# NWC-CUAHSI-Summer-Institute/LGAR-py

Measured on AMD Instinct MI355X. Metric: column-timesteps/sec, higher is better.
Workload: dtype f32

## Files before the change

### lgar_py_amd/csrc/lgar_column.hpp

```cpp
#pragma once
#include "lgar_geff.hpp"

namespace lgar {

template <typename R> struct Glob {
  R dt_h, initial_psi, pdm, wp_psi, frozen;
  R giuh[LGAR_GMAX];
  int nint, nsub, ng, bottom_mode, closed_form;
  long long iter_cap;
};

#define LGAR_COOP_GROUPS 16
template <typename S, int FMAX, int STRIDE = WAVE> struct FrontsView {
  S *base;
  unsigned char *fl;
  __device__ __forceinline__ S &Z(int i) const { return base[(0 * FMAX + i) * STRIDE]; }
  __device__ __forceinline__ S &TH(int i) const { return base[(1 * FMAX + i) * STRIDE]; }
  __device__ __forceinline__ S &PS(int i) const { return base[(2 * FMAX + i) * STRIDE]; }
  __device__ __forceinline__ S &DZ(int i) const { return base[(3 * FMAX + i) * STRIDE]; }
  __device__ __forceinline__ unsigned char &flag(int i) const { return fl[i * STRIDE]; }
  __device__ __forceinline__ int layer(int i) const { return fl[i * STRIDE] & 0x7f; }
  __device__ __forceinline__ bool bottom(int i) const { return (fl[i * STRIDE] & LGAR_FLAG_BOTTOM) != 0; }
  __device__ __forceinline__ void set_flag(int i, int layer, bool bottom) const {
    fl[i * STRIDE] = (unsigned char)(layer | (bottom ? LGAR_FLAG_BOTTOM : 0));
  }
  __device__ __forceinline__ void copy(int dst, int src) const {
    Z(dst) = Z(src); TH(dst) = TH(src); PS(dst) = PS(src); DZ(dst) = DZ(src);
    fl[dst * STRIDE] = fl[src * STRIDE];
  }
};

constexpr int MODE_LITERAL = 0, MODE_FAST = 1, MODE_MIXED = 3, MODE_COOP = 4, MODE_MIXED_COOP = 6;

template <typename S, int MODE> struct ModeTraits : ScalarKind<S> {
  using K = ScalarKind<S>;
  static constexpr bool literal = MODE == MODE_LITERAL;
  static constexpr bool mixed = MODE == MODE_MIXED || MODE == MODE_MIXED_COOP;
  static constexpr bool coop = MODE == MODE_COOP || MODE == MODE_MIXED_COOP;
  static constexpr bool mixed_f64 = mixed && K::plain_f64;
  static constexpr bool coop_f64 = coop && K::plain_f64;
  static constexpr int pol = (literal && K::f64) ? POL_LIBRARY : (!literal && K::plain_f32) ? POL_RCP32 : mixed_f64 ? POL_MIXED : POL_LEAN;
  static constexpr int stride = coop ? LGAR_COOP_GROUPS : WAVE;
  static constexpr bool giuh_mem = MODE == MODE_MIXED && !K::dual;
  static constexpr bool late_forcing_sums = MODE == MODE_MIXED;
  static constexpr bool fused_walk = !literal && !coop;
};

template <typename S, int NL, int FMAX, int MODE> struct Column {
  using R = real_t<S>;
  using M = ModeTraits<S, MODE>;
  static constexpr int POL = M::pol;
  const ColParams<S, NL> &P;
  const LGAR_KARG Glob<R> *G;
  FrontsView<S, FMAX, M::stride> F;
  int nf;
  int status;
  S ponded_water, previous_precip, ending_volume;
  S giuh_q[LGAR_GMAX];
  static constexpr int DEAD = LGAR_ST_BOTTOM | LGAR_ST_OVERFLOW | LGAR_ST_STRUCT;
  R *giuh_mem = nullptr;
  size_t giuh_stride = 0;
  bool giuh_live = false;
  S k_deepest;
  bool new_front_frozen;
  S memo_theta, memo_g;
  int memo_layer = -1;
  unsigned near_sat_fronts = 0u;
  S post_mass;
  bool post_mass_valid = false;
  bool post_event = false;
  bool psi_rewritten = false;
  S aet_psi_wp_memo;
  bool aet_psi_wp_known = false;
  bool count_geff = false;
  int share_lanes = 0;
  R *xchg = nullptr;
  int coop_rank = 0;
  int cap = FMAX;
  S a_precip, a_pet, a_aet, a_infil, a_runoff, a_perc, a_giuh, a_disch;

  __device__ Column(const ColParams<S, NL> &p, const LGAR_KARG Glob<R> *g, const FrontsView<S, FMAX, M::stride> &f) : P(p), G(g), F(f) {}

  __device__ __forceinline__ S cum_at(int k) const { return sel<S, NL>(P.cum, k); }
  __device__ __forceinline__ S capillary_drive(const LayerK<S> &lk, S theta1, S theta2, int site = 0, CoopRiders *riders = nullptr) {
    (void)site; (void)riders;
    LGAR_MEASURE_POINT(NOGEFF, lk, theta1, theta2)
    LGAR_COUNT_GEFF_CALL(site)
    LGAR_MEASURE_POINT(DUP_GEFF, lk, theta1, theta2)
    if constexpr (M::literal && M::f64) {
      return G->closed_form ? geff_closed<S, POL>(lk, theta1, theta2) : geff_literal<S, POL>(lk, theta1, theta2, G->nint);
    }
    if constexpr (M::dual && M::f64 && !M::literal) {
      if (share_lanes >= 2 && !G->closed_form) return geff_fused<S>(lk, theta1, theta2, G->nint, xchg, share_lanes);
    }
    if constexpr (M::coop_f64 && !M::mixed) {
      if (share_lanes > 1 && !G->closed_form) return geff_fused<S>(lk, theta1, theta2, G->nint, xchg, share_lanes, coop_rank, riders);
    }
    if constexpr (M::coop_f64 && M::mixed) {
      if (share_lanes > 1 && !G->closed_form)
        return geff_mixed_coop(val(lk.alpha), val(lk.n), val(lk.m), val(lk.inv_m), val(lk.inv_n), val(lk.ksat), val(lk.te), val(lk.tr),
                               theta1, theta2, G->nint, xchg, share_lanes, coop_rank);
    }
    if constexpr (M::mixed_f64) {
      if (!G->closed_form)
        return geff_mixed(val(lk.alpha), val(lk.n), val(lk.m), val(lk.inv_m), val(lk.inv_n), val(lk.ksat), val(lk.te), val(lk.tr),
                          theta1, theta2, G->nint);
    }
#ifndef LGAR_NO_F32_RARE_GEFF
    if constexpr (M::plain_f32 && !M::literal) {
      if (site != 1 && !G->closed_form)
        return geff_f32_rare(lk.alpha, lk.n, lk.m, lk.inv_m, lk.inv_n, lk.te, lk.tr, theta1, theta2, G->nint);
    }
#endif
    return G->closed_form ? geff_closed<S, POL>(lk, theta1, theta2) : geff(lk, theta1, theta2, G->nint);
  }
  __device__ __forceinline__ double capillary_drive_fronts(const LayerK<double> &lk, double theta1, double theta2, double psi1,
                                                           double psi2, double &kr_end) {
    LGAR_MEASURE_POINT(NOGEFF_FRONTS, lk, theta1, theta2, kr_end)
    LGAR_COUNT_GEFF_CALL(1)
    if constexpr (M::coop && M::mixed) {
      if (share_lanes > 1) return geff_mixed_heads<true>(lk, theta1, theta2, psi1, psi2, G->nint, kr_end, xchg, share_lanes, coop_rank);
    }
    return geff_mixed_heads(lk, theta1, theta2, psi1, psi2, G->nint, kr_end);
  }
  __device__ __forceinline__ S cum_prev(int k) const {
    S r = S(R(0.0));
#pragma unroll
    for (int j = 0; j < NL - 1; j++) {
      const S cj = P.cum[j];
      r = choose(k == j + 1, cj, r);
    }
    return r;
  }

  __device__ __forceinline__ bool feq(int a, int b) const {
    return val(F.Z(a)) == val(F.Z(b)) && val(F.PS(a)) == val(F.PS(b)) && val(F.DZ(a)) == val(F.DZ(b));
  }
  __device__ __forceinline__ void fdel(int i) {
    for (int j = i; j < nf - 1; j++) F.copy(j, j + 1);
    nf--;
  }
  __device__ __forceinline__ void range_of(int k, int &lo, int &len) const {
    lo = -1; len = 0;
    for (int i = 0; i < nf; i++)
      if (F.layer(i) == k) { if (len == 0) lo = i; len++; }
  }

  static constexpr int SCAN = 8;
  struct Rows {
    R z[SCAN], th[SCAN];
    int fl[SCAN];
  };
  __device__ __forceinline__ void fetch_rows(Rows &r) const {
#pragma unroll
    for (int q = 0; q < SCAN; q++) {
      r.z[q] = val(F.Z(q));
      r.th[q] = val(F.TH(q));
      r.fl[q] = F.flag(q);
    }
  }

  __device__ __forceinline__ S mass_balance() const {
    S ls[NL];
    if constexpr (M::coop_f64) {
      if (nf <= SCAN) {
        Rows r;
        fetch_rows(r);
#pragma unroll
        for (int j = 0; j < NL; j++) ls[j] = S(R(0.0));
#pragma unroll
        for (int q = 0; q < SCAN; q++) {
          const bool on = q < nf;
          const int lay = r.fl[q] & 0x7f;
          const bool next_same = (q + 1 < nf) && ((r.fl[(q + 1 < SCAN) ? q + 1 : q] & 0x7f) == lay);
          const R dth = next_same ? r.th[q] - r.th[(q + 1 < SCAN) ? q + 1 : q] : r.th[q];
          R base = R(0.0);
#pragma unroll
          for (int j = 1; j < NL; j++) base = choose(lay == j, val(P.cum[j]) - val(P.thick[j]), base);
          const R term = (r.z[q] - base) * dth;
#pragma unroll
          for (int j = 0; j < NL; j++) ls[j] = choose(on && lay == j, ls[j] + term, ls[j]);
        }
        S tot = ls[NL - 1];
#pragma unroll
        for (int j = NL - 2; j >= 0; j--) tot = ls[j] + tot;
        return tot;
      }
    }
    int i = 0;
#pragma unroll
    for (int j = 0; j < NL; j++) {
      S base = (j == 0) ? S(R(0.0)) : P.cum[j] - P.thick[j];
      S sum = S(R(0.0));
      while (i < nf && F.layer(i) == j) {
        bool next_same = (i + 1 < nf) && (F.layer(i + 1) == j);
        S dth = next_same ? (F.TH(i) - F.TH(i + 1)) : F.TH(i);
        sum = sum + (F.Z(i) - base) * dth;
        i++;
      }
      ls[j] = sum;
    }
    S tot = ls[NL - 1];
#pragma unroll
    for (int j = NL - 2; j >= 0; j--) tot = ls[j] + tot;
    return tot;
  }

  __device__ __forceinline__ S mass_and_events(bool &ev) const {
    S ls[NL];
    bool e = false;
    int i = 0;
#pragma unroll
    for (int j = 0; j < NL; j++) {
      S base = (j == 0) ? S(R(0.0)) : P.cum[j] - P.thick[j];
      S sum = S(R(0.0));
      while (i < nf && F.layer(i) == j) {
        const bool has_next = i + 1 < nf;
        const int fn = has_next ? F.flag(i + 1) : 0;
        const bool next_same = has_next && ((fn & 0x7f) == j);
        const S zi = F.Z(i), ti = F.TH(i);
        if (has_next) {
          const S zn = F.Z(i + 1), tn = F.TH(i + 1);
          e = e || (next_same && !(fn & LGAR_FLAG_BOTTOM) && val(zi) > val(zn));
          e = e || (next_same && val(ti) <= val(tn));
          e = e || (val(zi) > val(P.cum[j]));
          sum = sum + (zi - base) * (next_same ? (ti - tn) : ti);
        } else {
          sum = sum + (zi - base) * ti;
        }
        i++;
      }
      ls[j] = sum;
    }
    S tot = ls[NL - 1];
#pragma unroll
    for (int j = NL - 2; j >= 0; j--) tot = ls[j] + tot;
    ev = e;
    return tot;
  }

  __device__ __forceinline__ int free_drainage_front() const {
    R psi = val(F.PS(0));
    int idx = 0;
    for (int i = 0; i < nf; i++) {
      R pi = val(F.PS(i));
      if (pi <= psi) { psi = pi; idx = i; }
      else if (ab(pi - psi) <= R(1e-8) + R(1e-5) * ab(psi)) { psi = pi; idx = i; }
    }
    return idx;
  }

  __device__ __forceinline__ static void theta_slope(R alpha, R n, R m, R te, R tr, R psi, R &th, R &dth) {
    R ap = pwp<POL>(alpha * psi, n);
    R one_ap = R(1.0) + ap;
    R op = pwp<POL>(one_ap, m);
    R span = dv<POL>(R(1.0), op) * (te - tr);
    th = span + tr;
    dth = (psi > R(0.0)) ? dv<POL>(-(span * m * n * ap), psi * one_ap) : R(0.0);
  }

  __device__ __forceinline__ static void theta_slope2(R alpha, R n, R m, R te, R tr, R psi, R &th, R &dth, R &d2th) {
    R ap = pwp<POL>(alpha * psi, n);
    R one_ap = R(1.0) + ap;
    R op = pwp<POL>(one_ap, m);
    R span = dv<POL>(R(1.0), op) * (te - tr);
    th = span + tr;
    const R r = (psi > R(0.0)) ? dv<POL>(R(1.0), psi * one_ap) : R(0.0);
    dth = -(span * m * n * ap) * r;
    d2th = dth * ((n - R(1.0)) - n * ap) * r;
  }

  struct FirstEval {
    bool have = false;
    R M = R(0.0), dM = R(0.0), d2M = R(0.0);
    R thk = R(0.0);
    __device__ __forceinline__ void add(R thick, R th, R below, R dth, R d2th) {
      M += thick * (th - below);
      dM += thick * dth;
      d2M += thick * d2th;
    }
  };

  template <int K>
  __device__ __forceinline__ S theta_mass_balance_newton_f32(const LayerK<S> &lk, S psi0, S new_mass, S prior_mass,
                                                             const S (&dth)[NL], const S (&dthick)[NL], S dth_k, S dthick_k) {
// ... 464 lines not shown
          S psi_old = oc_ps;
          S psi = F.PS(i);
          S base = P.cum[NL - 2];
          S prior_mass = (oc_z - base) * (oc_th - R(0.0));
          S new_mass = (z - base) * (F.TH(i) - R(0.0));
          FirstEval fe;
#pragma unroll
          for (int j = 0; j < NL - 1; j++) {
            const LayerK<S> lj = pick_static(P, j);
            if constexpr (M::f64) {
              S theta;
              if constexpr (!M::dual) {
                R th, dt, d2;
                theta_slope2(val(lj.alpha), val(lj.n), val(lj.m), val(lj.te), val(lj.tr), val(psi), th, dt, d2);
                fe.add(val(P.thick[j]), th, R(0.0), dt, d2);
                theta = S(th);
              } else {
                theta = theta_from_h<S, POL>(lj, psi);
              }
              prior_mass = prior_mass + P.thick[j] * (theta - R(0.0));
              new_mass = new_mass + P.thick[j] * (theta - R(0.0));
            } else {
              S theta_old = theta_from_h<S, POL>(lj, psi_old);
              prior_mass = prior_mass + P.thick[j] * (theta_old - R(0.0));
              S theta = theta_from_h<S, POL>(lj, psi);
              new_mass = new_mass + P.thick[j] * (theta - R(0.0));
            }
            dthick[j] = P.thick[j];
          }
          if constexpr (M::plain_f64) {
            R tk, dk, ek;
            theta_slope2(val(lk.alpha), val(lk.n), val(lk.m), val(lk.te), val(lk.tr), val(psi), tk, dk, ek);
            fe.add(val(z) - val(base), tk, R(0.0), dk, ek);
            fe.thk = tk;
            fe.have = true;
          }
          if (F.layer(c.fdd) == NL - 1) prior_mass = prior_mass + c.infiltration - (R(0.0) + c.aet);
          S theta_new = theta_mass_balance<NL - 1>(lk, psi, new_mass, prior_mass, dth, dthick, S(R(0.0)), z - base, fe);
          F.TH(i) = mn(theta_new, lk.te);
          need_psi = true;
        }
      }
      if (need_psi) F.PS(i) = h_from_se<S, POL>(lk, se_from_theta(lk, F.TH(i)));
      LGAR_MEASURE_POINT(CLK, 24)
      c.on_z = oc_z; c.on_th = oc_th; c.on_ps = oc_ps;
      c.i = i - 1;
    }
  }
  template <int K> __device__ __forceinline__ void sweep_from(SweepCarry &c) {
    sweep_layer<K>(c);
    if constexpr (K > 0) sweep_from<K - 1>(c);
  }

  __device__ __forceinline__ void move_sweep(S infiltration, S aet, S old_mass, int fdd) {
    SweepCarry c;
    c.i = nf - 1; c.nf0 = nf; c.fdd = fdd;
    c.infiltration = infiltration; c.aet = aet;
    c.on_z = c.on_th = c.on_ps = S(R(0.0));
    c.near_sat = 0u;
    sweep_from<NL - 1>(c);
    near_sat_fronts = c.near_sat;
    if constexpr (!M::fused_walk) {
      check_column_mass(fdd, old_mass, infiltration, aet);
    } else {
      const S theta_e_k1 = sel<S, NL>(P.te, F.layer(fdd));
      const S mass_timestep = (old_mass + infiltration) - (aet + R(0.0));
      bool stepped = false, literal = false;
      if (__builtin_expect(ab(val(F.TH(fdd)) - val(theta_e_k1)) < Tol<R>::mass, 0)) {
        const S current_mass = mass_balance();
        const R err = ab(val(current_mass) - val(mass_timestep));
        if (ab(err - Tol<R>::mass) > Tol<R>::mass) {
          const bool nxt_same = (fdd + 1 < nf) && (F.layer(fdd + 1) == F.layer(fdd));
          const R slope = nxt_same ? val(F.TH(fdd)) - val(F.TH(fdd + 1)) : val(F.TH(fdd));
          if (slope > R(0.0)) {
            F.Z(fdd) = F.Z(fdd) + dv<POL>(val(mass_timestep) - val(current_mass), slope);
            stepped = true;
          } else {
            literal = true;
          }
        }
      }
      if (__builtin_expect(literal, 0)) check_column_mass(fdd, old_mass, infiltration, aet);
      post_mass = mass_and_events(post_event);
      if (stepped) {
        const R err = ab(val(post_mass) - val(mass_timestep));
        if (__builtin_expect(ab(err - Tol<R>::mass) > Tol<R>::mass, 0)) {
          check_column_mass(fdd, old_mass, infiltration, aet);
          post_mass = mass_and_events(post_event);
        }
      }
      post_mass_valid = true;
    }
  }

  __device__ __forceinline__ void merge_fronts() {
    int i = 0, lo = 0;
    while (i < nf - 1) {
      const int k = F.layer(i);
      if (i > 0 && F.layer(i - 1) != k) lo = i;
      const int nx = i + 1;
      const bool passing = (val(F.Z(i)) > val(F.Z(nx))) && (F.layer(nx) == k) && !F.bottom(nx);
      if (!passing) { i++; continue; }
      const int nn = i + 2;
      if (nn >= nf) { status |= LGAR_ST_STRUCT; return; }
      const LayerK<S> lk = pick(P, k);
      S mass = F.Z(i) * (F.TH(i) - F.TH(nx)) + F.Z(nx) * (F.TH(nx) - F.TH(nn));
      F.Z(i) = mass / (F.TH(i) - F.TH(nn));
      S se = se_from_theta(lk, F.TH(i));
      F.PS(i) = h_from_se<S, POL>(lk, se);
      int j = lo;
      while (j < nf && F.layer(j) == k && !feq(j, nx)) j++;
      if (j < nf && F.layer(j) == k) fdel(j);
      i = lo;
      while (i < nf && F.layer(i) == k) i++;
      lo = i;
    }
  }

  __device__ __forceinline__ void cross_layer_boundary() {
    int i = 0;
    while (i < nf - 1) {
      const int k = F.layer(i);
      const int nx = i + 1, nn = i + 2;
      const S cumk = cum_at(k);
      if (!(val(F.Z(i)) > val(cumk) && val(F.Z(nx)) == val(cumk))) { i++; continue; }
      if (k == NL - 1) {
        if (G->bottom_mode == 0) { status |= LGAR_ST_BOTTOM; return; }
        i++;
        continue;
      }
      if (nn >= nf) { status |= LGAR_ST_STRUCT; return; }
      const LayerK<S> lk = pick(P, k);
      const LayerK<S> ln = pick(P, k + 1);
      S overshot = F.Z(i) - F.Z(nx);
      S se = se_from_theta(lk, F.TH(i));
      F.PS(i) = h_from_se<S, POL>(lk, se);
// ... 73 lines not shown
#pragma unroll
    for (int j = NL - 2; j >= 0; j--) tot = ls[j] + tot;
    return tot;
  }

  __device__ __forceinline__ void update_psi() {
    for (int i = 0; i < nf - 1; i++) {
      const LayerK<S> lk = pick(P, F.layer(i));
      F.PS(i) = h_from_se<S, POL>(lk, se_from_theta(lk, F.TH(i)));
    }
  }

  __device__ __forceinline__ S front_k(int i, const LayerK<S> &lk) const {
    S k = k_from_se<S, POL>(lk, se_from_theta(lk, F.TH(i)));
    if (i == 0 && new_front_frozen) k = k * G->frozen;
    return k;
  }

  __device__ __forceinline__ bool front_event_pending() const {
    bool ev = false;
    S z1 = F.Z(0), t1 = F.TH(0);
    int f1 = F.flag(0);
    for (int i = 0; i + 1 < nf; i++) {
      const S z2 = F.Z(i + 1), t2 = F.TH(i + 1);
      const int f2 = F.flag(i + 1);
      const bool same = ((f1 ^ f2) & 0x7f) == 0;
      ev = ev || (same && !(f2 & LGAR_FLAG_BOTTOM) && val(z1) > val(z2));
      ev = ev || (same && val(t1) <= val(t2));
      ev = ev || (val(z1) > val(cum_at(f1 & 0x7f)));
      z1 = z2; t1 = t2; f1 = f2;
    }
    return ev;
  }

  __device__ __forceinline__ S move_wetting_front(S infiltration, S &aet, S old_mass, int fdd) {
    move_sweep(infiltration, aet, old_mass, fdd);
    LGAR_MEASURE_POINT(CLK, 3)
    S bottom_flux = S(R(0.0));
    LGAR_MEASURE_POINT(DUP_EVENT)
    bool pending;
    if constexpr (M::fused_walk) pending = post_event;
    else pending = front_event_pending();
    if (__builtin_expect(pending, 0)) {
      post_mass_valid = false;
      psi_rewritten = false;
      for (int pass = 0; pass < 2; pass++) {
        merge_fronts();
        if (pass == 0) cross_layer_boundary();
      }
      if (G->bottom_mode != 0) bottom_flux = cross_domain_boundary();
      S mass_change = fix_dry_over_wet();
      if (ab(val(mass_change)) > R(1e-7)) aet = aet - mass_change;
      if constexpr (!M::literal) { if (psi_rewritten || near_sat_fronts != 0u) update_psi(); }
    } else if constexpr (!M::literal && M::f64) {
      if (__builtin_expect(near_sat_fronts != 0u, 0)) {
        for (int i = 0; i < nf - 1; i++)
          if (near_sat_fronts & (1u << i)) {
            const LayerK<S> lk = pick(P, F.layer(i));
            F.PS(i) = h_from_se<S, POL>(lk, se_from_theta(lk, F.TH(i)));
          }
      }
    }
    if constexpr (M::literal) update_psi();
    LGAR_MEASURE_POINT(CLK, 4)
    LGAR_MEASURE_POINT(DUP_PSI)
    return bottom_flux;
  }

  __device__ __forceinline__ int calc_dzdt_pairs(S h_p) {
    const int hl = share_lanes >> 1;
    const bool upper = coop_rank >= hl;
    const int r2 = upper ? coop_rank - hl : coop_rank;
    R *tab2 = xchg + (upper ? LGAR_COOP_TAB_ROW : 0);
    int i = -1;
    auto next_moving = [&]() {
      while (++i < nf - 1) {
        if (F.bottom(i)) { F.DZ(i) = S(R(0.0)); continue; }
        const bool top = F.layer(i) == 0;
        if (top && val(F.TH(i + 1)) > val(F.TH(i))) status |= LGAR_ST_THETA_ORDER;
        if (val(F.TH(i) - F.TH(i + 1)) > R(0.0)) return i;
        F.DZ(i) = S(R(0.0));
      }
      return -1;
    };
    for (;;) {
      const int ia = next_moving();
      if (ia < 0) return i;
      const int ib = next_moving();
      const int ka = F.layer(ia), kb = (ib >= 0) ? F.layer(ib) : 0;
      if (ib < 0 || hl < 5 + ((ka > kb) ? ka : kb)) return ia - 1;
      const int im = upper ? ib : ia;
      const int k = upper ? kb : ka;
      const LayerK<S> lk = pick(P, k);
      const S theta_1 = F.TH(im + 1), theta_2 = F.TH(im);
      CoopRiders riders;
      {
        const int e = r2 - 5;
        LayerK<S> le = lk;
        S th_e = theta_2;
#pragma unroll
        for (int j = 0; j < NL - 1; j++) {
          const bool mine = (e == j) && (j < k);
          le.alpha = choose(mine, P.alpha[j], le.alpha); le.n = choose(mine, P.n[j], le.n); le.m = choose(mine, P.m[j], le.m);
          le.inv_m = choose(mine, P.inv_m[j], le.inv_m); le.ksat = choose(mine, P.ksat[j], le.ksat);
          le.te = choose(mine, P.te[j], le.te); le.tr = choose(mine, P.tr[j], le.tr);
        }
// ... 79 lines not shown
      const LayerK<S> lk = pick(P, k);
      LGAR_COUNT_GEFF_CALL(1)
      LGAR_COUNT_GEFF_CALL(1)
      double kr_mine;
      const S g_mine = geff_mixed_heads<true>(lk, F.TH(im + 1), F.TH(im), F.PS(im + 1), F.PS(im), G->nint, kr_mine, tab2, hl, r2);
      tab2[0] = g_mine;
      tab2[1] = kr_mine;
#pragma unroll
      for (int j = 0; j < NL - 1; j++)
        if (j < kmax) {
          const LayerK<S> lj = pick_static(P, j);
          const S tl = theta_from_h<S, POL>(lj, F.PS(im));
          tab2[2 + j] = k_from_se<S, POL>(lj, se_from_theta(lj, tl));
        }
      lds_exchange_point();
      S g2[2];
      R kr2[2], kk[2][NL];
#pragma unroll
      for (int h = 0; h < 2; h++) {
        g2[h] = xchg[h * 64];
        kr2[h] = xchg[h * 64 + 1];
#pragma unroll
        for (int j = 0; j < NL - 1; j++) kk[h][j] = xchg[h * 64 + 2 + j];
      }
      lds_exchange_point();
#pragma unroll
      for (int h = 0; h < 2; h++) {
        const int f = h ? ib : ia;
        const int kf = h ? kb : ka;
        const LayerK<S> lf = pick(P, kf);
        const S g = g2[h];
        S ki = lf.ksat * kr2[h];
        if (f == 0 && new_front_frozen) ki = ki * G->frozen;
        if (is_nan(val(g))) status |= LGAR_ST_NAN;
        const S delta_theta = F.TH(f) - F.TH(f + 1);
        S dzdt;
        if (kf == 0) {
          dzdt = dv<POL>(S(R(1.0)), delta_theta) * (dv<POL>(lf.ksat * (g + h_p), F.Z(f)) + ki);
        } else {
          S den = S(R(0.0)) + dv<POL>(F.Z(f) - cum_prev(kf), ki);
#pragma unroll
          for (int j = 0; j < NL - 1; j++)
            if (j < kf) {
              S pt = (j != 0) ? P.cum[(j > 0) ? j - 1 : 0] : S(R(0.0));
              den = den + dv<POL>(P.cum[j] - pt, S(kk[h][j]));
            }
          dzdt = dv<POL>(S(R(1.0)), delta_theta) * (dv<POL>(F.Z(f), den) + dv<POL>(lf.ksat * (g + h_p), F.Z(f)));
        }
        F.DZ(f) = dzdt;
      }
    }
  }

  __device__ __forceinline__ void calc_dzdt(S h_p) {
    int i = -1;
    if constexpr (M::coop_f64 && M::mixed) {
      if (share_lanes >= 4 && !G->closed_form) i = calc_dzdt_pairs_mixed(h_p);
    }
    if constexpr (M::coop_f64 && !M::mixed) {
      if (share_lanes >= LGAR_COOP_PAIR_LANES && !G->closed_form) i = calc_dzdt_pairs(h_p);
    }
    for (;;) {
      bool found = false;
      while (!found && ++i < nf - 1) {
        if (F.bottom(i)) { F.DZ(i) = S(R(0.0)); continue; }
        const bool top = F.layer(i) == 0;
        if (top && val(F.TH(i + 1)) > val(F.TH(i))) status |= LGAR_ST_THETA_ORDER;
        if (val(F.TH(i) - F.TH(i + 1)) > R(0.0)) found = true;
        else F.DZ(i) = S(R(0.0));
      }
      if (any_lane(found) == 0ull) break;
      LGAR_MEASURE_POINT(CLK, 10)
      if (found) {
        const int k = F.layer(i);
        const LayerK<S> lk = pick(P, k);
        S theta_1 = F.TH(i + 1), theta_2 = F.TH(i);
        S delta_theta = F.TH(i) - F.TH(i + 1);
        S g, ki;
        bool fronts_done = false;
        if constexpr (M::mixed_f64) {
          if (!G->closed_form) {
            double kr_end;
            g = capillary_drive_fronts(lk, theta_1, theta_2, F.PS(i + 1), F.PS(i), kr_end);
            ki = lk.ksat * kr_end;
            if (i == 0 && new_front_frozen) ki = ki * G->frozen;
            fronts_done = true;
          }
        }
        CoopRiders riders;
        if constexpr (M::coop_f64 && !M::mixed) {
          if (!G->closed_form && share_lanes >= 5 + k) {
            const int e = coop_rank - 5;
            LayerK<S> le = lk;
            S th_e = F.TH(i);
            if (k > 0) {
#pragma unroll
              for (int j = 0; j < NL - 1; j++) {
                const bool mine = (e == j) && (j < k);
                le.alpha = choose(mine, P.alpha[j], le.alpha); le.n = choose(mine, P.n[j], le.n); le.m = choose(mine, P.m[j], le.m);
                le.inv_m = choose(mine, P.inv_m[j], le.inv_m); le.ksat = choose(mine, P.ksat[j], le.ksat);
                le.te = choose(mine, P.te[j], le.te); le.tr = choose(mine, P.tr[j], le.tr);
              }
              const S tl = theta_from_h<S, POL>(le, F.PS(i));
              th_e = choose(e >= 0 && e < k, tl, th_e);
            }
            riders.n = 1 + k;
            riders.l = le;
// ... 171 lines not shown
  }

  __device__ __forceinline__ void drain() {
    a_precip = a_pet = a_aet = a_infil = a_runoff = a_perc = a_giuh = a_disch = S(R(0.0));
  }

  __device__ __forceinline__ void forward(S precip, S pet) {
    const R dt = G->dt_h;
    if (is_nan(val(precip)) || is_nan(val(pet))) status |= LGAR_ST_NAN;
    S ending_volume_sub = ending_volume;
    for (int sub = 0; sub < G->nsub; sub++) {
      if (status & DEAD) return;
      new_front_frozen = false;
      post_mass_valid = false;
      S precip_sub = precip * dt;
      S pet_sub = pet * dt;
      S ponded_depth_sub = precip_sub + ponded_water;
      S ponded_water_sub = S(R(0.0)), runoff_sub = S(R(0.0)), infiltration_sub = S(R(0.0)), AET_sub = S(R(0.0));
      const bool create = (val(previous_precip) == R(0.0)) && (val(precip_sub) > R(0.0)) && (val(ponded_water) == R(0.0));
      LGAR_MEASURE_POINT(CLK, 0)
      LGAR_MEASURE_POINT(DUP_FDD)
      const int fdd = free_drainage_front();
      const bool saturated = val(F.TH(0)) >= val(P.te[0]);
      if (val(pet) > R(0.0)) {
        if (!aet_psi_wp_known) {
          aet_psi_wp_memo = aet_psi_wp<S, POL>(pick_static(P, 0), G->wp_psi);
          aet_psi_wp_known = true;
        }
        AET_sub = aet_from_psi_wp<S, POL>(pet, dt, F.PS(0), aet_psi_wp_memo);
      }
      if constexpr (!M::late_forcing_sums) {
        a_precip = a_precip + precip_sub;
        a_pet = a_pet + ((val(pet_sub) > R(0.0)) ? pet_sub : S(R(0.0)));
      }
      const bool inserting = !create && val(ponded_depth_sub) > R(0.0);
      LGAR_MEASURE_POINT(CLK, 1)
      if (inserting) {
        LGAR_ABLATABLE(INSERT, insert_water(fdd, precip_sub, ponded_depth_sub, infiltration_sub, runoff_sub);)
        a_infil = a_infil + infiltration_sub;
        a_runoff = a_runoff + runoff_sub;
        ponded_water_sub = ponded_depth_sub;
      }
      LGAR_MEASURE_POINT(CLK, 2)
      if (!create || !saturated) {
        S perc_sub = S(R(0.0));
        LGAR_ABLATABLE(MOVE, perc_sub = move_wetting_front(create ? S(R(0.0)) : infiltration_sub, AET_sub, ending_volume_sub, fdd);)
        if (!create) a_perc = a_perc + perc_sub;
      }
      if (__builtin_expect(create && !saturated, 0)) {
        S dry_depth = calc_dry_depth();
        create_surficial_front(dry_depth, ponded_depth_sub, infiltration_sub);
        a_infil = a_infil + infiltration_sub;
        post_mass_valid = false;
      }
      if (!inserting) {
        if (val(ponded_depth_sub) < G->pdm) {
          runoff_sub = S(R(0.0));
          ponded_water_sub = ponded_depth_sub;
          ponded_depth_sub = S(R(0.0));
        } else {
          runoff_sub = ponded_depth_sub - G->pdm;
          ponded_depth_sub = S(G->pdm);
          ponded_water_sub = ponded_depth_sub;
          a_runoff = a_runoff + runoff_sub;
        }
      }
      LGAR_MEASURE_POINT(CLK, 5)
      LGAR_ABLATABLE(DZDT, calc_dzdt(ponded_depth_sub);)
      LGAR_MEASURE_POINT(CLK, 6)
      LGAR_MEASURE_POINT(DUP_DZDT, ponded_depth_sub)
      LGAR_MEASURE_POINT(DUP_MB, ending_volume_sub)
      if constexpr (M::fused_walk) {
        if (__builtin_expect(!post_mass_valid, 0)) post_mass = mass_balance();
        ending_volume_sub = post_mass;
      } else {
        ending_volume_sub = mass_balance();
      }
      LGAR_MEASURE_POINT(CLK, 7)
      previous_precip = precip_sub;
      ending_volume = ending_volume_sub;
      if constexpr (M::late_forcing_sums) {
        a_precip = a_precip + precip_sub;
        a_pet = a_pet + ((val(pet_sub) > R(0.0)) ? pet_sub : S(R(0.0)));
      }
      a_aet = a_aet + AET_sub;
      ponded_water = ponded_water_sub;
      if constexpr (M::giuh_mem) {
        if (giuh_live || val(runoff_sub) > R(0.0)) {
          const int ng = G->ng;
          S q[LGAR_GMAX];
#pragma unroll
          for (int i = 0; i < LGAR_GMAX; i++) q[i] = (i < ng) ? S(giuh_mem[(size_t)i * giuh_stride]) : S(R(0.0));
#pragma unroll
          for (int i = 0; i < LGAR_GMAX; i++) if (i < ng) q[i] = q[i] + (G->giuh[i] * runoff_sub);
          const S now = q[0];
          R qsum = R(0.0);
#pragma unroll
          for (int i = 0; i < LGAR_GMAX; i++) {
            const S shifted = (i + 1 < LGAR_GMAX) ? q[(i + 1 < LGAR_GMAX) ? i + 1 : i] : S(R(0.0));
            qsum += val(shifted);
            if (i < ng) giuh_mem[(size_t)i * giuh_stride] = val(shifted);
          }
          giuh_live = qsum > R(0.0);
          a_giuh = a_giuh + now;
          a_disch = a_disch + now;
        }
// ... 29 lines not shown
```

### lgar_py_amd/csrc/lgar_forward_body.hpp

```cpp
#pragma once
#include "lgar_column.hpp"

namespace lgar {

template <typename R> struct KArgs {
  int N, T, F;
  int Nf, Fg;
  int coop;
  unsigned *ticket;
  int chain_first, chain_last;
  const unsigned *pending_in;
  unsigned *pending_out;
  const R *alpha, *n, *ksat, *theta_e, *theta_r, *thick;
  R *depth, *theta, *psi, *k, *dzdt;
  uint8_t *flags;
  int32_t *nf;
  R *scalars;
  R *totals;
  const R *precip, *pet;
  R *series[LGAR_NACC];
  double *basin;
  const R *weights;
  unsigned basin_mask;
  int32_t *status;
// ... 137 lines not shown
  for (int j = 0; j < LGAR_NACC; j++) a.totals[j * N + c] = (j == 9) ? col.ending_volume : R(0);
}

template <typename R, int NL, int FMAX, int MODE, int MAPPED = -1>
__device__ __forceinline__ void forward_lane(const LGAR_KARG KArgs<R> *ap, size_t c, bool live, int lane,
                                             ForwardLDS<R, FMAX, MODE> &lds, bool leader = true, R *xchg = nullptr, int group = 0,
                                             int rank = 0) {
  using M = ModeTraits<R, MODE>;
  const LGAR_KARG KArgs<R> &a = *ap;
  const size_t N = (size_t)a.N;
  const bool basin_on = (a.basin != nullptr) && (a.basin_mask != 0u);
  int status = a.status[c];
  int t_begin = live ? 0 : a.T;
  if (!a.chain_first) {
    t_begin = (live && (status & LGAR_ST_RESUME)) ? (int)((unsigned)status >> LGAR_ST_STEP_SHIFT) : a.T;
    if (any_lane(t_begin < a.T) == 0ull) return;
  }
  status &= LGAR_ST_FAULT_MASK;
  LGAR_MEASURE_POINT(POISON_LDS, lds, M::coop ? group : lane)
  ColParams<R, NL> P;
  load_params<R, NL>(a, c, P);
  const int slot = M::coop ? group : lane;
  Column<R, NL, FMAX, MODE> col(P, &ap->G, make_view<R, FMAX, M::stride>(&lds.f[0][0][0], &lds.fl[0][0], slot));
  const int nf_stored = a.nf[c];
  const int cap = FMAX < a.F ? FMAX : a.F;
  int nf = nf_stored < 0 ? 0 : (nf_stored > cap ? cap : nf_stored);
  const int nf_before = nf;
  col.nf = nf;
  for (int i = 0; i < nf; i++) {
    col.F.Z(i) = a.depth[i * N + c];
    col.F.TH(i) = a.theta[i * N + c];
    col.F.PS(i) = a.psi[i * N + c];
    col.F.DZ(i) = a.dzdt[i * N + c];
    col.F.flag(i) = a.flags[i * N + c];
  }
  col.ponded_water = a.scalars[0 * N + c];
  col.previous_precip = a.scalars[1 * N + c];
  col.ending_volume = a.scalars[2 * N + c];
  if constexpr (M::giuh_mem) {
    col.giuh_mem = &a.scalars[3 * N + c];
    col.giuh_stride = N;
    R qsum = R(0);
#pragma unroll
    for (int i = 0; i < LGAR_GMAX; i++) qsum += a.scalars[(3 + i) * N + c];
    col.giuh_live = qsum > R(0);
  } else {
#pragma unroll
    for (int i = 0; i < LGAR_GMAX; i++) col.giuh_q[i] = a.scalars[(3 + i) * N + c];
  }
  col.status = status;
  if (nf < NL) col.status |= LGAR_ST_STRUCT;
  col.k_deepest = (nf > 0) ? a.k[(size_t)(nf - 1) * N + c] : R(0);
  col.new_front_frozen = false;
  col.cap = FMAX < a.F ? FMAX : a.F;
  col.count_geff = a.counters != nullptr;
  col.share_lanes = (xchg != nullptr) ? a.coop : 0;
  col.xchg = xchg;
  col.coop_rank = rank;
  col.drain();
  constexpr int SR = LdsSums<R, FMAX>::rows;
  R tot[8];
#pragma unroll
  for (int j = 0; j < 8; j++) {
    tot[j] = R(0);
    if (j < SR) lds.sums[j][slot] = R(0);
  }
  double wgt = 0.0;
  if (basin_on && leader) wgt = a.weights ? (double)a.weights[c] : 1.0;

  constexpr bool PARK = M::f64 && (FMAX <= LGAR_CAP_SMALL) && !M::coop;
  LaneInt<PARK> t_stop_at;
  bool overflow_on_load = false;
  {
    int t_stop = a.T;
    if (t_begin < a.T && nf_stored > cap) {
      if constexpr (PARK) t_stop = a.chain_last ? -1 : t_begin;
      else if (a.chain_last) { overflow_on_load = true; t_stop = -1; } else t_stop = t_begin;
    }
    t_stop_at.set(t_stop);
  }
  if constexpr (PARK) overflow_on_load = t_begin < a.T && nf_stored > cap && a.chain_last;
  if (overflow_on_load) {
    col.status |= LGAR_ST_OVERFLOW;
    if constexpr (FMAX == LGAR_FMAX) {
      if (leader)
        for (int t = t_begin; t < a.T; t++)
#pragma unroll
          for (int j = 0; j < LGAR_NACC; j++)
            if (a.series[j]) a.series[j][(size_t)t * N + c] = R(0);
    }
  }
  unsigned series_mask = 0u;
#pragma unroll
  for (int j = 0; j < LGAR_NACC; j++)
    if (a.series[j]) series_mask |= 1u << j;
  const int T = a.T;
  const size_t Nf = (size_t)a.Nf;
  size_t cf;
  if (MAPPED < 0 ? (a.fmap != nullptr) : (MAPPED != 0)) {
    const int m = a.fmap[c / (size_t)a.Fg];
    cf = (size_t)(m < 0 ? 0 : (m < a.Nf ? m : a.Nf - 1));
  } else {
    cf = (Nf == N) ? c : (c / (size_t)a.Fg) % Nf;
  }
  constexpr bool AHEAD = M::coop;
  R precip_ahead = R(0), pet_ahead = R(0);
// ... 123 lines not shown
```

### lgar_py_amd/csrc/lgar_measure.hpp

```cpp
#pragma once
#ifdef LGAR_NO_F32_REUSE
#define LGAR_NO_DZDT_MEMO
#define LGAR_NO_F32_RARE_GEFF
#define LGAR_NO_GEFF_ENDS
#endif

__device__ __forceinline__ float opaque(float x) { asm volatile("" : "+v"(x)); return x; }
__device__ __forceinline__ double opaque(double x) { asm volatile("" : "+v"(x)); return x; }

#define LGAR_MEASURE_POINT(NAME, ...) LGAR_POINT_##NAME(__VA_ARGS__)
#define LGAR_ABLATABLE(NAME, ...) LGAR_STMT_##NAME(__VA_ARGS__)

#ifdef LGAR_ABL_NOINSERT
#define LGAR_STMT_INSERT(...)
#else
#define LGAR_STMT_INSERT(...) __VA_ARGS__
#endif
#ifdef LGAR_ABL_NOMOVE
#define LGAR_STMT_MOVE(...)
#else
#define LGAR_STMT_MOVE(...) __VA_ARGS__
#endif
#ifdef LGAR_ABL_NODZDT
#define LGAR_STMT_DZDT(...)
#else
#define LGAR_STMT_DZDT(...) __VA_ARGS__
#endif

#ifdef LGAR_ABL_NOGEFF
#define LGAR_POINT_NOGEFF(lk, theta1, theta2) return theta1 * theta2 + lk.alpha;
#else
#define LGAR_POINT_NOGEFF(lk, theta1, theta2)
#endif
#ifdef LGAR_ABL_NOGEFF
#define LGAR_POINT_NOGEFF_FRONTS(lk, theta1, theta2, kr) { kr = theta1; return theta1 * theta2 + lk.alpha; }
#else
#define LGAR_POINT_NOGEFF_FRONTS(lk, theta1, theta2, kr)
#endif
#ifdef LGAR_COUNT_SITE
#define LGAR_COUNT_IF_SITE(site) if (site == LGAR_COUNT_SITE)
#else
#define LGAR_COUNT_IF_SITE(site)
#endif
#ifdef LGAR_COUNT_MAXLANES
#define LGAR_COUNT_IF_SPARSE if (__builtin_popcountll(any_lane(true)) <= LGAR_COUNT_MAXLANES)
#else
#define LGAR_COUNT_IF_SPARSE
#endif
#ifdef LGAR_COUNT_LANES
#define LGAR_COUNT_WHO count_geff
#else
#define LGAR_COUNT_WHO (count_geff && first_active_lane())
#endif
#define LGAR_COUNT_GEFF_CALL(site) \
  LGAR_COUNT_IF_SITE(site) LGAR_COUNT_IF_SPARSE { if (LGAR_COUNT_WHO) status += (1 << LGAR_ST_STEP_SHIFT); }
#ifdef LGAR_DUP_GEFF
#define LGAR_POINT_DUP_GEFF(lk, theta1, theta2)                                                    \
  if constexpr (!M::dual) {                                                                         \
    const S extra = geff(lk, opaque(theta1), opaque(theta2), G->nint);                             \
    if (val(extra) == R(12345.678)) return extra;  \
  }
#else
#define LGAR_POINT_DUP_GEFF(lk, theta1, theta2)
#endif

#ifdef LGAR_ABL_NOSEARCH
#define LGAR_POINT_NOSEARCH(lk, psi, new_mass) return theta_from_h<S, POL>(lk, psi + new_mass);
#else
#define LGAR_POINT_NOSEARCH(lk, psi, new_mass)
#endif
#ifdef LGAR_DUP_SEARCH
#define LGAR_POINT_DUP_SEARCH(K, lk, psi, new_mass, prior_mass, dth, dthick, dth_k, dthick_k)      \
  if constexpr (!M::dual) {                                                                         \
    const S extra = theta_mass_balance<K>(lk, opaque(psi), opaque(new_mass), opaque(prior_mass), dth, dthick, dth_k, dthick_k); \
    if (val(extra) == R(-1.0)) status |= LGAR_ST_STRUCT;                           \
  }
#else
#define LGAR_POINT_DUP_SEARCH(...)
#endif

#ifdef LGAR_DUP_EVENT
#define LGAR_POINT_DUP_EVENT()                                                                     \
  if (front_event_pending() && val(F.Z(0)) == R(-12345.0)) status |= LGAR_ST_STRUCT;  \
  asm volatile("" ::: "memory");
#else
#define LGAR_POINT_DUP_EVENT()
#endif
#ifdef LGAR_DUP_PSI
#define LGAR_POINT_DUP_PSI() asm volatile("" ::: "memory"); update_psi();
#else
#define LGAR_POINT_DUP_PSI()
#endif
#ifdef LGAR_DUP_FDD
#define LGAR_POINT_DUP_FDD()                                                                       \
  if (free_drainage_front() == 12345) status |= LGAR_ST_STRUCT;                    \
  asm volatile("" ::: "memory");
#else
#define LGAR_POINT_DUP_FDD()
#endif
#ifdef LGAR_DUP_DZDT
#define LGAR_POINT_DUP_DZDT(h_p) asm volatile("" ::: "memory"); calc_dzdt(h_p);
#else
#define LGAR_POINT_DUP_DZDT(h_p)
#endif
#ifdef LGAR_DUP_MB
#define LGAR_POINT_DUP_MB(volume)                                                                  \
  volume = mass_balance();                                                                         \
  asm volatile("" ::: "memory");                                                                   \
// ... 90 lines not shown
```

### lgar_py_amd/csrc/lgar_scalar.hpp

```cpp
#pragma once
#ifndef LGAR_DEVSIM
#include <hip/hip_runtime.h>
#endif
#include <stdint.h>

#include "../../include/lgar.h"
#include "lgar_math.hpp"

#ifndef LGAR_DEVSIM
#define LGAR_KARG __attribute__((address_space(4)))
#else
#define LGAR_KARG
#endif

namespace lgar {

constexpr int WAVE = 64;

template <typename S> struct Real { using type = S; };
template <typename S> using real_t = typename Real<S>::type;
template <typename S> struct ScalarKind {
  using R = real_t<S>;
  static constexpr bool f64 = sizeof(R) == 8;
  static constexpr bool f32 = !f64;
// ... 47 lines not shown
template <typename S, int POL> __device__ __forceinline__ S pwq(const S &x, const S &y) {
  if constexpr (!ScalarKind<S>::dual) return pwp<POL>(x, y);
  else return pwx<POL == POL_LIBRARY>(x, y);
}

#ifndef LGAR_DEVSIM
__device__ __forceinline__ float rcp32(float b) { return __builtin_amdgcn_rcpf(b); }
#else
__device__ __forceinline__ float rcp32(float b) { return 1.0f / b; }
#endif
template <int POL> __device__ __forceinline__ float dv(float a, float b) {
  if constexpr (POL == POL_RCP32) return a * rcp32(b);
  return a / b;
}
#ifndef LGAR_DEVSIM
__device__ __forceinline__ double lean_div(double a, double b) {
  double r = __builtin_amdgcn_rcp(b);
  r = __builtin_fma(__builtin_fma(-b, r, 1.0), r, r);
  const double q = a * r;
  double res = __builtin_fma(__builtin_fma(-b, q, a), r, q);
  if (__builtin_expect(res != res, 0)) res = a / b;
  return res;
}
#else
__device__ __forceinline__ double lean_div(double a, double b) { return a / b; }
#endif
template <int POL> __device__ __forceinline__ double dv(double a, double b) {
  if constexpr (POL == POL_LEAN || POL == POL_MIXED) return lean_div(a, b);
  return a / b;
}
__device__ __forceinline__ double lg2(double x) { return fast_log2<false>(x); }
__device__ __forceinline__ double ex2(double x) { return fast_exp2<false>(x); }
__device__ __forceinline__ double lg2e(double x) { return fast_log2<true>(x); }
__device__ __forceinline__ double ex2e(double x) { return fast_exp2<true>(x); }
__device__ __forceinline__ float lg2p(float x) { return lg2(x); }
__device__ __forceinline__ float ex2p(float x) { return ex2(x); }
__device__ __forceinline__ double lg2p(double x) { return fast_log2_core<false>(x); }
__device__ __forceinline__ double ex2p(double x) { return fast_exp2_core<false, false>(x); }
__device__ __forceinline__ double sq(double x) { return sqrt(x); }
__device__ __forceinline__ double ab(double x) { return fabs(x); }
__device__ __forceinline__ float ab(float x) { return fabsf(x); }
__device__ __forceinline__ double mn(double a, double b) { return fmin(a, b); }
__device__ __forceinline__ float mn(float a, float b) { return fminf(a, b); }
__device__ __forceinline__ bool is_nan(double x) { return x != x; }
__device__ __forceinline__ bool is_nan(float x) { return x != x; }
__device__ __forceinline__ bool same_bits(double a, double b) { return a == b; }
__device__ __forceinline__ bool same_bits(float a, float b) { return a == b; }

#ifdef LGAR_MEASURE
#include "lgar_measure.hpp"
#else
#define LGAR_MEASURE_POINT(NAME, ...)
#define LGAR_ABLATABLE(NAME, ...) __VA_ARGS__
#define LGAR_COUNT_GEFF_CALL(site) \
  if (count_geff && first_active_lane()) status += (1 << LGAR_ST_STEP_SHIFT);
#endif

template <typename R> struct Tol;
template <> struct Tol<double> {
  static constexpr double mass = 1e-12;
  static constexpr double nochange = 1e-15;
  static constexpr double tiny = 1e-50;
};
template <> struct Tol<float> {
  static constexpr float mass = 2e-5f;
  static constexpr float nochange = 1e-9f;
  static constexpr float tiny = 1e-30f;
};

template <typename S> struct LayerK {
  S alpha, n, m, inv_m, inv_n, ksat, te, tr;
};

template <typename S> __device__ __forceinline__ void derive_layer(const S &n, S &m, S &inv_m, S &inv_n) {
  using R = real_t<S>;
  m = R(1.0) - (R(1.0) / n);
  inv_m = R(1.0) / m;
  inv_n = R(1.0) / n;
}

template <typename S, int NL> struct ColParams {
  S alpha[NL], n[NL], m[NL], inv_m[NL], inv_n[NL], ksat[NL], te[NL], tr[NL], thick[NL], cum[NL];
};

__device__ __forceinline__ float choose(bool c, float a, float b) { return c ? a : b; }
__device__ __forceinline__ double choose(bool c, double a, double b) { return c ? a : b; }

template <typename S, int NL> __device__ __forceinline__ S sel(const S (&a)[NL], int k) {
  S v[NL];
#pragma unroll
  for (int j = 0; j < NL; j++) v[j] = a[j];
  S r = v[0];
#pragma unroll
  for (int j = 1; j < NL; j++) r = choose(k == j, v[j], r);
  return r;
}

template <typename S, int NL> __device__ __forceinline__ LayerK<S> pick(const ColParams<S, NL> &P, int k) {
  LayerK<S> l;
  l.alpha = sel<S, NL>(P.alpha, k);
  l.n = sel<S, NL>(P.n, k);
  l.m = sel<S, NL>(P.m, k);
  l.ksat = sel<S, NL>(P.ksat, k);
  l.inv_m = sel<S, NL>(P.inv_m, k);
  l.inv_n = sel<S, NL>(P.inv_n, k);
  l.te = sel<S, NL>(P.te, k);
  l.tr = sel<S, NL>(P.tr, k);
  return l;
// ... 10 lines not shown
```

Measured before the change: 12.68 billion.

## Add top-layer-only fast path for sweep, dz/dt and mass balance

Adds a per-column flag, updated when fronts change, that marks columns whose extra wetting fronts all sit in the top layer and whose deeper layers hold only their bottom front. When every lane in a wave has this shape, the front sweep, dz/dt computation and mass/event check run specialized versions that use static top-layer parameters and skip per-front layer selection and multi-layer denominators. This cuts divergent layer lookups and branching for the common structure, at the cost of a layout scan after each structural change, extra wave votes, and more code that can raise register pressure.

```diff
diff --git a/lgar_py_amd/csrc/lgar_column.hpp b/lgar_py_amd/csrc/lgar_column.hpp
--- a/lgar_py_amd/csrc/lgar_column.hpp
+++ b/lgar_py_amd/csrc/lgar_column.hpp
@@ -44,11 +44,20 @@
   static constexpr bool giuh_mem = MODE == MODE_MIXED && !K::dual;
   static constexpr bool late_forcing_sums = MODE == MODE_MIXED;
   static constexpr bool fused_walk = !literal && !coop;
+#ifndef LGAR_NO_TOP_LAYER_STEP
+  static constexpr bool top_step = K::plain_f32 && !literal;
+#else
+  static constexpr bool top_step = false;
+#endif
 };
 
-template <typename S, int NL, int FMAX, int MODE> struct Column {
+template <bool ON> struct TopTableFlag { bool top_table = false; };
+template <> struct TopTableFlag<false> { static constexpr bool top_table = false; };
+
+template <typename S, int NL, int FMAX, int MODE> struct Column : TopTableFlag<ModeTraits<S, MODE>::top_step> {
   using R = real_t<S>;
   using M = ModeTraits<S, MODE>;
+  using TopTableFlag<M::top_step>::top_table;
   static constexpr int POL = M::pol;
   const ColParams<S, NL> &P;
   const LGAR_KARG Glob<R> *G;
@@ -146,6 +155,16 @@
       if (F.layer(i) == k) { if (len == 0) lo = i; len++; }
   }
 
+  __device__ __forceinline__ bool is_top_table() const {
+    const int m = nf - NL;
+    bool t = m >= 1;
+    for (int i = 0; i < nf; i++) {
+      const int f = F.flag(i);
+      t = t && (f == ((i < m) ? 0 : ((i - m) | LGAR_FLAG_BOTTOM)));
+    }
+    return t;
+  }
+
   static constexpr int SCAN = 8;
   struct Rows {
     R z[SCAN], th[SCAN];
@@ -231,6 +250,38 @@
         i++;
       }
       ls[j] = sum;
+    }
+    S tot = ls[NL - 1];
+#pragma unroll
+    for (int j = NL - 2; j >= 0; j--) tot = ls[j] + tot;
+    ev = e;
+    return tot;
+  }
+
+  __device__ __forceinline__ S mass_and_events_top(bool &ev) const {
+    const int m = nf - NL;
+    S ls[NL];
+    bool e = false;
+    const S base0 = S(R(0.0));
+    S sum = S(R(0.0));
+    S zi = F.Z(0), ti = F.TH(0);
+    for (int i = 0; i < m; i++) {
+      const S zn = F.Z(i + 1), tn = F.TH(i + 1);
+      e = e || (i + 1 < m && val(zi) > val(zn));
+      e = e || (val(ti) <= val(tn));
+      e = e || (val(zi) > val(P.cum[0]));
+      sum = sum + (zi - base0) * (ti - tn);
+      zi = zn; ti = tn;
+    }
+    e = e || (val(zi) > val(P.cum[0]));
+    sum = sum + (zi - base0) * ti;
+    ls[0] = sum;
+#pragma unroll
+    for (int j = 1; j < NL; j++) {
+      const S base = P.cum[j] - P.thick[j];
+      const S z = F.Z(m + j), t = F.TH(m + j);
+      if (j < NL - 1) e = e || (val(z) > val(P.cum[j]));
+      ls[j] = S(R(0.0)) + (z - base) * t;
     }
     S tot = ls[NL - 1];
 #pragma unroll
@@ -801,13 +852,61 @@
     if constexpr (K > 0) sweep_from<K - 1>(c);
   }
 
+  template <int K> __device__ __forceinline__ void sweep_top_boundary(int i) {
+    const LayerK<S> lk = pick_static(P, K);
+    const bool fresh = same_bits(F.PS(i), F.PS(i + 1));
+    if (!fresh) {
+      S ap;
+      F.TH(i) = theta_from_h_ap<S, POL>(lk, F.PS(i + 1), ap);
+      F.PS(i) = F.PS(i + 1);
+    }
+    if constexpr (K > 0) sweep_top_boundary<K - 1>(i - 1);
+  }
+  __device__ __forceinline__ void sweep_top(const SweepCarry &c) {
+    const LayerK<S> lk = pick_static(P, 0);
+    const int m = c.nf0 - NL;
+    S on_th = F.TH(m);
+    sweep_top_boundary<NL - 2>(m + NL - 2);
+    for (int i = m - 1; i >= 0; i--) {
+      const S oc_z = F.Z(i), oc_th = F.TH(i);
+      if (feq(i, m)) {
+        const bool fresh = same_bits(F.PS(i), F.PS(i + 1));
+        if (!fresh) {
+          S ap;
+          F.TH(i) = theta_from_h_ap<S, POL>(lk, F.PS(i + 1), ap);
+          F.PS(i) = F.PS(i + 1);
+        }
+      } else {
+        S prior_mass = oc_z * (oc_th - on_th);
+        if (i == c.fdd || feq(c.fdd, i)) prior_mass = prior_mass + (c.infiltration - (R(0.0) + c.aet));
+        S z = F.Z(i) + (F.DZ(i) * G->dt_h);
+        z = mn(z, P.cum[NL - 1]);
+        F.Z(i) = z;
+        const bool zero_dzdt = ab(val(F.DZ(i))) <= R(1e-8);
+        if (!zero_dzdt) {
+          S potential = dv<POL>(prior_mass, z) + F.TH(i + 1);
+          F.TH(i) = mn(lk.te, potential);
+        }
+        F.PS(i) = h_from_se<S, POL>(lk, se_from_theta(lk, F.TH(i)));
+      }
+      on_th = oc_th;
+    }
+  }
+
   __device__ __forceinline__ void move_sweep(S infiltration, S aet, S old_mass, int fdd) {
     SweepCarry c;
     c.i = nf - 1; c.nf0 = nf; c.fdd = fdd;
     c.infiltration = infiltration; c.aet = aet;
     c.on_z = c.on_th = c.on_ps = S(R(0.0));
     c.near_sat = 0u;
-    sweep_from<NL - 1>(c);
+    if constexpr (M::top_step) {
+      const bool fast = any_lane(!top_table) == 0ull;
+      LGAR_COUNT_TOP_STEP(fast)
+      if (fast) sweep_top(c);
+      else sweep_from<NL - 1>(c);
+    } else {
+      sweep_from<NL - 1>(c);
+    }
     near_sat_fronts = c.near_sat;
     if constexpr (!M::fused_walk) {
       check_column_mass(fdd, old_mass, infiltration, aet);
@@ -830,7 +929,12 @@
         }
       }
       if (__builtin_expect(literal, 0)) check_column_mass(fdd, old_mass, infiltration, aet);
-      post_mass = mass_and_events(post_event);
+      if constexpr (M::top_step) {
+        if (any_lane(!top_table) == 0ull) post_mass = mass_and_events_top(post_event);
+        else post_mass = mass_and_events(post_event);
+      } else {
+        post_mass = mass_and_events(post_event);
+      }
       if (stepped) {
         const R err = ab(val(post_mass) - val(mass_timestep));
         if (__builtin_expect(ab(err - Tol<R>::mass) > Tol<R>::mass, 0)) {
@@ -1010,6 +1114,7 @@
       S mass_change = fix_dry_over_wet();
       if (ab(val(mass_change)) > R(1e-7)) aet = aet - mass_change;
       if constexpr (!M::literal) { if (psi_rewritten || near_sat_fronts != 0u) update_psi(); }
+      if constexpr (M::top_step) top_table = is_top_table();
     } else if constexpr (!M::literal && M::f64) {
       if (__builtin_expect(near_sat_fronts != 0u, 0)) {
         for (int i = 0; i < nf - 1; i++)
@@ -1195,7 +1300,82 @@
     }
   }
 
+  __device__ __forceinline__ void calc_dzdt_top_step(S h_p) {
+    const bool fast = any_lane(!top_table) == 0ull;
+    const int m = nf - NL;
+    int i = -1;
+    for (;;) {
+      bool found = false;
+      if (fast) {
+        while (!found && ++i < m) {
+          if (val(F.TH(i + 1)) > val(F.TH(i))) status |= LGAR_ST_THETA_ORDER;
+          if (val(F.TH(i) - F.TH(i + 1)) > R(0.0)) found = true;
+          else F.DZ(i) = S(R(0.0));
+        }
+      } else {
+        while (!found && ++i < nf - 1) {
+          if (F.bottom(i)) { F.DZ(i) = S(R(0.0)); continue; }
+          const bool top = F.layer(i) == 0;
+          if (top && val(F.TH(i + 1)) > val(F.TH(i))) status |= LGAR_ST_THETA_ORDER;
+          if (val(F.TH(i) - F.TH(i + 1)) > R(0.0)) found = true;
+          else F.DZ(i) = S(R(0.0));
+        }
+      }
+      if (any_lane(found) == 0ull) break;
+      LGAR_MEASURE_POINT(CLK, 10)
+      if (found) {
+        int k = 0;
+        LayerK<S> lk;
+        if (fast) {
+          lk = pick_static(P, 0);
+        } else {
+          k = F.layer(i);
+          lk = pick(P, k);
+        }
+        S theta_1 = F.TH(i + 1), theta_2 = F.TH(i);
+        S delta_theta = F.TH(i) - F.TH(i + 1);
+        S g, ki;
+        bool fronts_done = false;
+        LGAR_MEASURE_POINT(F32_HEADS_FROM_PSI, lk, i, g, ki, fronts_done)
+        if (!fronts_done) {
+          g = capillary_drive(lk, theta_1, theta_2, 1);
+          ki = front_k(i, lk);
+#ifndef LGAR_NO_DZDT_MEMO
+          if (same_bits(theta_2, lk.te) && (i == 0 || (!fast && F.layer(i - 1) != k))) { memo_theta = theta_1; memo_g = g; memo_layer = k; }
+#endif
+        }
+        if (is_nan(val(g))) status |= LGAR_ST_NAN;
+        S dzdt;
+        if (fast || k == 0) {
+          dzdt = dv<POL>(S(R(1.0)), delta_theta) * (dv<POL>(lk.ksat * (g + h_p), F.Z(i)) + ki);
+        } else {
+          S den = S(R(0.0)) + dv<POL>(F.Z(i) - cum_prev(k), ki);
+#pragma unroll
+          for (int j = 0; j < NL - 1; j++)
+            if (j < k) {
+              const LayerK<S> lj = pick_static(P, j);
+              S tl = theta_from_h<S, POL>(lj, F.PS(i));
+              S kl = k_from_se<S, POL>(lj, se_from_theta(lj, tl));
+              S pt = (j != 0) ? P.cum[(j > 0) ? j - 1 : 0] : S(R(0.0));
+              den = den + dv<POL>(P.cum[j] - pt, kl);
+            }
+          dzdt = dv<POL>(S(R(1.0)), delta_theta) * (dv<POL>(F.Z(i), den) + dv<POL>(lk.ksat * (g + h_p), F.Z(i)));
+        }
+        F.DZ(i) = dzdt;
+        LGAR_MEASURE_POINT(CLK, 17)
+      }
+    }
+    if (fast) {
+#pragma unroll
+      for (int j = 0; j < NL - 1; j++) F.DZ(m + j) = S(R(0.0));
+    }
+  }
+
   __device__ __forceinline__ void calc_dzdt(S h_p) {
+    if constexpr (M::top_step) {
+      calc_dzdt_top_step(h_p);
+      return;
+    }
     int i = -1;
     if constexpr (M::coop_f64 && M::mixed) {
       if (share_lanes >= 4 && !G->closed_form) i = calc_dzdt_pairs_mixed(h_p);
@@ -1473,6 +1653,7 @@
         create_surficial_front(dry_depth, ponded_depth_sub, infiltration_sub);
         a_infil = a_infil + infiltration_sub;
         post_mass_valid = false;
+        if constexpr (M::top_step) top_table = is_top_table();
       }
       if (!inserting) {
         if (val(ponded_depth_sub) < G->pdm) {
diff --git a/lgar_py_amd/csrc/lgar_forward_body.hpp b/lgar_py_amd/csrc/lgar_forward_body.hpp
--- a/lgar_py_amd/csrc/lgar_forward_body.hpp
+++ b/lgar_py_amd/csrc/lgar_forward_body.hpp
@@ -213,6 +213,7 @@
   if (nf < NL) col.status |= LGAR_ST_STRUCT;
   col.k_deepest = (nf > 0) ? a.k[(size_t)(nf - 1) * N + c] : R(0);
   col.new_front_frozen = false;
+  if constexpr (M::top_step) col.top_table = col.is_top_table();
   col.cap = FMAX < a.F ? FMAX : a.F;
   col.count_geff = a.counters != nullptr;
   col.share_lanes = (xchg != nullptr) ? a.coop : 0;
diff --git a/lgar_py_amd/csrc/lgar_measure.hpp b/lgar_py_amd/csrc/lgar_measure.hpp
--- a/lgar_py_amd/csrc/lgar_measure.hpp
+++ b/lgar_py_amd/csrc/lgar_measure.hpp
@@ -52,8 +52,12 @@
 #else
 #define LGAR_COUNT_WHO (count_geff && first_active_lane())
 #endif
+#ifndef LGAR_COUNT_TOP_LAYER_STEP
 #define LGAR_COUNT_GEFF_CALL(site) \
   LGAR_COUNT_IF_SITE(site) LGAR_COUNT_IF_SPARSE { if (LGAR_COUNT_WHO) status += (1 << LGAR_ST_STEP_SHIFT); }
+#else
+#define LGAR_COUNT_GEFF_CALL(site)
+#endif
 #ifdef LGAR_DUP_GEFF
 #define LGAR_POINT_DUP_GEFF(lk, theta1, theta2)                                                    \
   if constexpr (!M::dual) {                                                                         \
diff --git a/lgar_py_amd/csrc/lgar_scalar.hpp b/lgar_py_amd/csrc/lgar_scalar.hpp
--- a/lgar_py_amd/csrc/lgar_scalar.hpp
+++ b/lgar_py_amd/csrc/lgar_scalar.hpp
@@ -123,8 +123,18 @@
 #else
 #define LGAR_MEASURE_POINT(NAME, ...)
 #define LGAR_ABLATABLE(NAME, ...) __VA_ARGS__
+#ifndef LGAR_COUNT_TOP_LAYER_STEP
 #define LGAR_COUNT_GEFF_CALL(site) \
   if (count_geff && first_active_lane()) status += (1 << LGAR_ST_STEP_SHIFT);
+#else
+#define LGAR_COUNT_GEFF_CALL(site)
+#endif
+#endif
+#ifdef LGAR_COUNT_TOP_LAYER_STEP
+#define LGAR_COUNT_TOP_STEP(fast) \
+  if (count_geff && first_active_lane() && (fast) == (LGAR_COUNT_TOP_LAYER_STEP != 0)) status += (1 << LGAR_ST_STEP_SHIFT);
+#else
+#define LGAR_COUNT_TOP_STEP(fast)
 #endif
 
 template <typename R> struct Tol;
```

After: 13.03 billion, median of 6. 1.03x the previous value.
